# david-cortes/poismf

Hardware: AMD Instinct MI355X
Metric: nonzeros/sec per full A+B sweep (higher is better)
Workload: dtype f32; 1 GPU; uniform 1000000x100000, 99949803 nnz (100000000 triplets, seed 1, duplicates summed), k=50, method=pg, maxupd=10, l2=1000, step=1e-09

## Files before the change

poismf_amd/csrc/poismf_hip.hip:

```cpp
#include <hip/hip_runtime.h>

#include <algorithm>
#include <atomic>
#include <cstdio>
#include <cstdlib>
#include <type_traits>

#include "plan.hpp"
#include "reg_eval.hpp"
#include "quad_eval.hpp"
#include "lane_eval.hpp"
#include "solvers.hpp"

#ifndef PMF_TU
#define PMF_TU -1
#endif
constexpr bool tu_has(int kmethod) { return PMF_TU == -1 || PMF_TU == kmethod; }

template <class EV, class = void> struct cold_constants : std::false_type {};
template <class EV> struct cold_constants<EV, std::void_t<decltype(EV::COLD_CONSTANTS)>> : std::integral_constant<bool, EV::COLD_CONSTANTS> {};

template <class EV, class = void> struct has_idle_tile : std::false_type {};
template <class EV> struct has_idle_tile<EV, std::void_t<decltype(&EV::idle_tile)>> : std::true_type {};

template <class EV, class T, int NC, int METHOD>
__device__ __forceinline__ void solve_row(const HalfArgs<T>& a, EV& ev, const T (&bs)[NC], unsigned lrow, unsigned nnz)
{
    const int k = a.geom.k;
    T* out = a.M + (size_t)(a.row_offset + lrow) * (size_t)k;
    T* out_p = a.Mp != nullptr ? a.Mp + (size_t)(a.row_offset + lrow) * (size_t)a.ldM : nullptr;
    T x[NC];
    if (nnz == 0) {
        T z = (T)0;
        asm volatile("" : "+v"(z));
        PMF_EW x[i] = z;
        ev.store_vec(out, x);
        if (out_p != nullptr) ev.store_vec(out_p, x);
        return;
    }
    ev.start_point(out, x);
    ev.n_eval = 0;

    T shift[NC];
    PMF_EW shift[i] = bs[i];
    const bool weighted = a.P.w != (T)1;
    if (weighted) {
        T cs[NC];
        PMF_EW cs[i] = (T)0;
        ev.tile_colsum(cs);
        T w_here = a.P.w;
        asm volatile("" : "+v"(w_here));
        const T wm1 = w_here - (T)1.;
        PMF_EW {
            shift[i] = cs[i] * wm1;
            shift[i] = shift[i] + bs[i];
        }
        if (METHOD == K_PG) {
            PMF_EW shift[i] = shift[i] * a.P.neg_step;
            if (a.P.neg_step2 != (T)1) { PMF_EW shift[i] = shift[i] * a.P.neg_step2; }
        }
    }

    SolveStats st;
    if constexpr (METHOD == K_EVAL) {
        T g[NC];
        double f;
        if (a.P.maxupd == 0) {
            f = (double)fun_single(ev, a.P, shift, x);
            grad_single(ev, a.P, shift, x, g, weighted);
        } else f = (double)fun_and_grad(ev, a.P, shift, x, g);
        ev.store_vec(out, g);
        if (out_p != nullptr) ev.store_vec(out_p, g);
        if (a.dec_rows != nullptr && ev.lane == 0 && ev.wid == 0 && ev.member == 0) {
            const unsigned long long fb = __builtin_bit_cast(unsigned long long, f);
            a.dec_rows[2 * (size_t)lrow] = (unsigned)fb;
            a.dec_rows[2 * (size_t)lrow + 1] = (unsigned)(fb >> 32);
        }
        return;
    } else if constexpr (METHOD == K_PG) {
        pg_row(ev, a.P, x, shift);
    } else if constexpr (METHOD == K_CG) {
        if constexpr (EV::MAY_CACHE) {
            if (a.P.limit_step && ev.pq_cap > 0 && nnz <= (unsigned)ev.pq_cap) cg_row_cached(ev, a.P, shift, x, weighted, st);
            else cg_row(ev, a.P, shift, x, weighted, st);
        } else cg_row(ev, a.P, shift, x, weighted, st);
    } else {
        T prev[NC];
        PMF_EW prev[i] = x[i];
        if (!a.reuse_prev) { PMF_EW x[i] = (T)1e-3; }
        (void)Tnc<T, NC, EV>::minimize(ev, a.P, shift, x, st);
        if (a.early_stop) {
            PMF_EW prev[i] = prev[i] - x[i];
            const T moved = ev.dot(prev, prev);
            if ((double)moved <= 1e-4 && ev.lane == 0 && ev.wid == 0 && ev.member == 0) atomicAdd(a.n_unchanged, 1u);
        }
    }
    ev.store_vec(out, x);
    if (out_p != nullptr) ev.store_vec(out_p, x);
#ifndef PMF_PROBE
    if (a.eval_rows != nullptr && ev.lane == 0 && ev.wid == 0 && ev.member == 0) a.eval_rows[lrow] += ev.n_eval;
#endif
    if (a.dec_rows != nullptr && ev.lane == 0 && ev.wid == 0 && ev.member == 0) {
        unsigned d0 = (unsigned)st.niter | ((unsigned)st.rc << 24), d1 = (unsigned)st.nfeval;
        if constexpr (cold_constants<EV>::value) asm volatile("" : "+v"(d0), "+v"(d1));
        a.dec_rows[2 * (size_t)lrow] = d0;
        a.dec_rows[2 * (size_t)lrow + 1] = d1;
    }
}

template <int METHOD, class T> __device__ __forceinline__ unsigned take_ticket(const HalfArgs<T>& a)
{
    unsigned st = 0u;
    if constexpr (METHOD != K_PG) {
        if (a.stop != nullptr) st = __hip_atomic_load(a.stop, __ATOMIC_RELAXED, __HIP_MEMORY_SCOPE_SYSTEM);
    }
    const unsigned t = atomicAdd(a.queue, 1u);
    return st != 0u ? 0xffffffffu : t;
}

template <class EV, class T, int NC, int METHOD, int NW>
__device__ __forceinline__ void sweep_rows(const HalfArgs<T>& a, EV& ev, unsigned char* smem)
{
    if (a.gate != nullptr && __hip_atomic_load(a.gate, __ATOMIC_RELAXED, __HIP_MEMORY_SCOPE_AGENT) == 0) return;
    ev.init(a.geom, a.F, smem);
    T bs[NC];
    ev.load_vec(a.bsum, bs);
    const RowDesc* desc = a.desc + a.perm_begin;
    if constexpr (EV::PIPELINED && (EV::PIPE_MW == 1 || (EV::PIPE_MW == 2 && METHOD == K_PG))) {
        unsigned r = blockIdx.x;
        auto ticket = [&]() -> unsigned {
            if (a.queue != nullptr) {
                if constexpr (NW > 1) {
                    unsigned* slot = ev.ticket_slot();
                    if (threadIdx.x == 0) *slot = take_ticket<METHOD>(a);
                    __syncthreads();
                    const unsigned t = uniform(*slot);
                    __syncthreads();
                    return t;
                }
                unsigned t = 0;
                if (ev.lane == 0) t = take_ticket<METHOD>(a);
                return uniform(t);
            }
            unsigned t = r;
            r += gridDim.x;
            if constexpr (METHOD != K_PG) {
                if (a.stop != nullptr && __hip_atomic_load(a.stop, __ATOMIC_RELAXED, __HIP_MEMORY_SCOPE_SYSTEM) != 0u) t = 0xffffffffu;
            }
            return t;
        };
        auto fetch = [&](unsigned t) -> RowDesc { return desc[t < a.nrows ? t : 0u]; };
        unsigned t0 = ticket(), t1 = ticket();
        RowDesc d0 = fetch(t0), d1 = fetch(t1);
        if (t0 < a.nrows) ev.fetch_meta(a.indices + (((unsigned long long)d0.p0_hi << 32) | d0.p0_lo), d0.nnz);
#ifdef PMF_PROBE
        unsigned probe_i = 0;
#endif
        while (t0 < a.nrows) {
            const unsigned long long p0 = ((unsigned long long)d0.p0_hi << 32) | d0.p0_lo;
            if (d0.nnz != 0) ev.gather(a.values + p0, d0.nnz);
            else if constexpr (has_idle_tile<EV>::value) ev.idle_tile();
            const unsigned t2 = ticket();
            const RowDesc d2 = fetch(t2);
            if (t1 < a.nrows) ev.fetch_meta(a.indices + (((unsigned long long)d1.p0_hi << 32) | d1.p0_lo), d1.nnz);
#ifdef PMF_PROBE
            ev.probe = (a.eval_rows != nullptr && blockIdx.x == 5 && threadIdx.x < WAVE && probe_i < 60) ? a.eval_rows + 16 * probe_i : nullptr;
            if (ev.probe != nullptr && ev.lane == 0) { ev.probe[10] = (unsigned)__builtin_amdgcn_s_memtime(); ev.probe[11] = d0.nnz; }
            probe_i++;
#endif
            solve_row<EV, T, NC, METHOD>(a, ev, bs, d0.lrow, d0.nnz);
            t0 = t1; d0 = d1;
            t1 = t2; d1 = d2;
        }
        return;
    } else {
        unsigned r = blockIdx.x;
        for (;;) {
            if (a.queue != nullptr) {
                if constexpr (NW > 1) {
                    unsigned* next_row = ev.ticket_slot();
                    if (threadIdx.x == 0) *next_row = take_ticket<METHOD>(a);
                    __syncthreads();
                    r = uniform(*next_row);
                    __syncthreads();
                } else {
                    unsigned t = 0;
                    if (ev.lane == 0) t = take_ticket<METHOD>(a);
                    r = uniform(t);
                }
            }
            if (r >= a.nrows) break;
            if constexpr (METHOD != K_PG) {
                if (a.queue == nullptr && a.stop != nullptr && uniform(__hip_atomic_load(a.stop, __ATOMIC_RELAXED, __HIP_MEMORY_SCOPE_SYSTEM)) != 0u) break;
            }
            const RowDesc d = desc[r];
            r += gridDim.x;
            const unsigned nnz = uniform(d.nnz);
            const unsigned long long p0 = ((unsigned long long)uniform(d.p0_hi) << 32) | uniform(d.p0_lo);
            if (nnz != 0) ev.begin_row(a.indices + p0, a.values + p0, nnz);
            solve_row<EV, T, NC, METHOD>(a, ev, bs, uniform(d.lrow), nnz);
        }
    }
}

template <class T, int NC, int METHOD, int SL, int NW>
__global__ __launch_bounds__(WAVE* NW) void half_sweep_kernel(const HalfArgs<T> a)
{
    extern __shared__ __attribute__((aligned(16))) unsigned char smem[];
    constexpr bool PF = SL > 0 && METHOD != K_TNCG;
    RowEval<T, NC, SL, NW, PF> ev;
    if constexpr (NW > 1) {
        if (a.arrive != nullptr && threadIdx.x == 0) atomicAdd(a.arrive, 1u);
    }
#ifdef PMF_TIMING
    const unsigned long long t_kernel = __builtin_amdgcn_s_memtime();
#endif
    sweep_rows<RowEval<T, NC, SL, NW, PF>, T, NC, METHOD, NW>(a, ev, smem);
#ifdef PMF_TIMING
    ev.tacc[5] = __builtin_amdgcn_s_memtime() - t_kernel;
    if (ev.lane == 0 && ev.wid == 0)
        for (int q = 0; q < 6; q++) atomicAdd(&g_pmf_timing[q], ev.tacc[q]);
#endif
}

template <class EV, class T, int NC, int METHOD>
__device__ __forceinline__ void team_rows(const HalfArgs<T>& a, EV& ev, unsigned char* smem)
{
    if (a.arrive != nullptr && threadIdx.x == 0) atomicAdd(a.arrive, 1u);
    ev.init(a.geom, a.F, smem);
    T bs[NC];
    ev.load_vec(a.bsum, bs);
    const RowDesc* desc = a.desc + a.perm_begin;
    const unsigned M = a.team_members;
    unsigned* box = ev.ticket_slot();
    if (threadIdx.x == 0) {
        const unsigned n = atomicAdd((unsigned*)a.team_buf, 1u);
        box[0] = n / M;
        box[1] = n % M;
    }
    __syncthreads();
    const unsigned team = uniform(box[0]);
    ev.member = (int)uniform(box[1]);
    __syncthreads();
    if ((size_t)(team + 1) * gt_team_words(M) + GT_HEAD_WORDS > GT_BUF_BYTES / 8) return;
    ev.tm_M = (int)M;
    ev.tm_seq = 0;
    ev.tm_words = a.team_buf + GT_HEAD_WORDS + (size_t)team * gt_team_words(M);
    ev.tm_err = a.team_err;
    ev.tm_spin = a.team_spin;
    unsigned long long* mail = ev.tm_words;
    constexpr unsigned END = 0xffffffffu;
    if (threadIdx.x == 0) atomicAdd((unsigned*)(mail + 2), 1u);
    if (a.team_spin <= 1u && threadIdx.x == 0) __hip_atomic_store(a.team_err, 1u, __ATOMIC_RELAXED, __HIP_MEMORY_SCOPE_AGENT);
    if (ev.wid == 0) {
        for (unsigned spins = 0;; spins++) {
            if (a.team_spin <= 1u) break;
            if (uniform((unsigned)gt_load(mail + 2)) >= M) break;
            if ((spins & 255u) == 255u) {
                if (uniform(__hip_atomic_load(a.team_err, __ATOMIC_RELAXED, __HIP_MEMORY_SCOPE_AGENT)) != 0) break;
                if (uniform(__hip_atomic_load(a.queue, __ATOMIC_RELAXED, __HIP_MEMORY_SCOPE_AGENT)) >= a.nrows) break;
            }
            if ((spins >> 6) > a.team_spin) { __hip_atomic_store(a.team_err, 1u, __ATOMIC_RELAXED, __HIP_MEMORY_SCOPE_AGENT); break; }
            __builtin_amdgcn_s_sleep(8);
        }
    }
    __syncthreads();
    for (unsigned rowno = 1;; rowno++) {
        if (ev.wid == 0) {
            unsigned tk = END;
            if (ev.member == 0) {
                unsigned t0 = 0;
                if (ev.lane == 0) t0 = take_ticket<METHOD>(a);
                tk = uniform(t0);
                if (tk >= a.nrows || uniform(__hip_atomic_load(a.team_err, __ATOMIC_RELAXED, __HIP_MEMORY_SCOPE_AGENT)) != 0) tk = END;
                gt_store(mail + (rowno & 1u), ((unsigned long long)rowno << 32) | tk);
            } else {
                unsigned seen = uniform(__hip_atomic_load(a.queue, __ATOMIC_RELAXED, __HIP_MEMORY_SCOPE_AGENT));
                for (unsigned spins = 0;; spins++) {
                    const unsigned long long v = gt_load(mail + (rowno & 1u));
                    const unsigned hi = uniform((unsigned)(v >> 32)), lo = uniform((unsigned)v);
                    if (hi == rowno) { tk = lo; break; }
                    if ((spins & 255u) == 255u) {
                        if (uniform(__hip_atomic_load(a.team_err, __ATOMIC_RELAXED, __HIP_MEMORY_SCOPE_AGENT)) != 0) break;
                        const unsigned q = uniform(__hip_atomic_load(a.queue, __ATOMIC_RELAXED, __HIP_MEMORY_SCOPE_AGENT));
                        if (q != seen) { seen = q; spins = 0; }
                        else if (rowno == 1u && q >= a.nrows) break;
                    }
                    if (spins > a.team_spin) { __hip_atomic_store(a.team_err, 1u, __ATOMIC_RELAXED, __HIP_MEMORY_SCOPE_AGENT); break; }
                    __builtin_amdgcn_s_sleep(4);
                }
            }
            box[0] = tk;
        }
        __syncthreads();
        const unsigned t = uniform(box[0]);
        __syncthreads();
        if (t >= a.nrows) break;
        const RowDesc d = desc[t];
        const unsigned nnz = uniform(d.nnz);
        const unsigned long long p0 = ((unsigned long long)uniform(d.p0_hi) << 32) | uniform(d.p0_lo);
        const unsigned S = ((nnz + M - 1u) / M + (EV::TEAM_ROUND - 1u)) / EV::TEAM_ROUND * EV::TEAM_ROUND;
        const unsigned off = (unsigned)ev.member * S;
        const unsigned mine = off < nnz ? (nnz - off < S ? nnz - off : S) : 0u;
        ev.begin_row(a.indices + p0 + (mine ? off : 0u), a.values + p0 + (mine ? off : 0u), mine);
        solve_row<EV, T, NC, METHOD>(a, ev, bs, uniform(d.lrow), nnz);
    }
}
template <class T, int NC, int METHOD, int SL, int NW>
__global__ __launch_bounds__(WAVE* NW) void half_sweep_giant_kernel(const HalfArgs<T> a)
{
    extern __shared__ __attribute__((aligned(16))) unsigned char smem[];
    constexpr bool PF = SL > 0 && METHOD != K_TNCG;
    using EV = RowEval<T, NC, SL, NW, PF, true>;
    EV ev;
    team_rows<EV, T, NC, METHOD>(a, ev, smem);
}
template <class T, int METHOD, int KS, int LV, int LA, int LL, int NW, int LP>
__global__ __launch_bounds__(WAVE* NW) __attribute__((amdgpu_waves_per_eu(1, 1))) void half_sweep_lane_team_kernel(const HalfArgs<T> a)
{
    using EV = LaneEval<T, KS, LV, LA, LL, NW, false, LP, 0, true>;
    __shared__ __attribute__((aligned(16))) unsigned char smem[EV::SMEM_BYTES];
    EV ev;
    team_rows<EV, T, EV::NC, METHOD>(a, ev, smem);
}

#ifndef PMF_PG_EXTRA
#define PMF_PG_EXTRA 56
#endif
#ifndef PMF_CG_EXTRA
#define PMF_CG_EXTRA 120
#endif
#ifndef PMF_TNC_EXTRA
#define PMF_TNC_EXTRA 100
#endif
constexpr int reg_waves(int tile_regs, int method)
{
    const int need = tile_regs + (method == K_PG ? PMF_PG_EXTRA : method == K_CG ? PMF_CG_EXTRA : PMF_TNC_EXTRA);
    for (int w : { 8, 6, 5, 4, 3, 2 })
        if ((512 / w) / 8 * 8 >= need) return w;
    return 1;
}
template <class T, int METHOD, int G, int NS> constexpr bool reg_pairs() { return METHOD == K_PG && sizeof(T) == 4 && G == 16 && NS == 1; }
template <class T, int METHOD, int S, int G, int NS>
__global__ __launch_bounds__(WAVE) __attribute__((amdgpu_waves_per_eu(reg_waves(4 * S * NS, METHOD)))) void half_sweep_reg_kernel(const HalfArgs<T> a)
{
    using EV = RegEval<T, S, G, NS, 1, 1, reg_pairs<T, METHOD, G, NS>()>;
    EV ev;
    constexpr int SMEM = EV::SMEM_BYTES;
    __shared__ __attribute__((aligned(16))) unsigned char smem[SMEM > 0 && METHOD == K_CG ? SMEM : 16];
#ifdef PMF_TIMING
    const unsigned long long t_kernel = __builtin_amdgcn_s_memtime();
#endif
    sweep_rows<EV, T, EV::NC, METHOD, 1>(a, ev, smem);
#ifdef PMF_TIMING
    if (ev.lane == 0) atomicAdd(&g_pmf_timing[5], __builtin_amdgcn_s_memtime() - t_kernel);
#endif
}

template <int Q>
__global__ __launch_bounds__(WAVE) __attribute__((amdgpu_waves_per_eu(reg_waves(QuadEval<Q>::TILE_REGS, K_PG)))) void half_sweep_quad_kernel(const HalfArgs<float> a)
{
    using EV = QuadEval<Q>;
    EV ev;
    sweep_rows<EV, float, EV::NC, K_PG, 1>(a, ev, nullptr);
}

constexpr int regw_waves(int tile_regs, int method, int nw)
{
    const int w = reg_waves(tile_regs + (method == K_PG ? 8 : 0), method);
    return nw >= 16 && w < 4 ? 4 : (nw >= 8 && w < 2 ? 2 : w);
}
template <class T, int METHOD, int S, int G, int NS, int NW>
__global__ __launch_bounds__(WAVE* NW) __attribute__((amdgpu_waves_per_eu(regw_waves(4 * S * NS, METHOD, NW)))) void half_sweep_regw_kernel(const HalfArgs<T> a)
{
    using EV = RegEval<T, S, G, NS, NW>;
    __shared__ __attribute__((aligned(16))) unsigned char smem[EV::SMEM_BYTES];
    EV ev;
    sweep_rows<EV, T, EV::NC, METHOD, NW>(a, ev, smem);
}

template <class T, int METHOD, int S, int G, int NS, int NW, int M>
__global__ __launch_bounds__(WAVE* NW) __attribute__((amdgpu_waves_per_eu(1))) void half_sweep_team_kernel(const HalfArgs<T> a)
{
    using EV = RegEval<T, S, G, NS, NW, M>;
    constexpr int NC = EV::NC;
    __shared__ __attribute__((aligned(16))) unsigned char smem[EV::SMEM_BYTES];
    EV ev;
    ev.init(a.geom, a.F, smem);
    T bs[NC];
    ev.load_vec(a.bsum, bs);
    const RowDesc* desc = a.desc + a.perm_begin;
    unsigned* arrive = (unsigned*)a.team_buf;
    unsigned* err = a.team_err;
    unsigned* box = ev.ticket_slot();
    if (threadIdx.x == 0) {
        unsigned xcc = 0;
        if (gridDim.x >= 8u * 4u * (unsigned)M) {
            asm volatile("s_getreg_b32 %0, hwreg(HW_REG_XCC_ID)" : "=s"(xcc));
            xcc &= 7u;
        }
        const unsigned n = atomicAdd(arrive + xcc, 1u);
        box[0] = xcc * TEAM_SLOTS_PER_XCD + n / (unsigned)M;
        box[1] = n % (unsigned)M;
        if (n / (unsigned)M >= TEAM_SLOTS_PER_XCD) __hip_atomic_store(err, 2u, __ATOMIC_RELAXED, __HIP_MEMORY_SCOPE_AGENT);
    }
    __syncthreads();
    const unsigned team = uniform(box[0]) % TEAM_SLOTS;
    ev.member = (int)uniform(box[1]);
    __syncthreads();
    ev.team_words = a.team_buf + TEAM_HEAD_WORDS + (size_t)team * TEAM_WORDS;
    ev.team_err = err;
    ev.team_spin = a.team_spin;
    unsigned long long* mail = ev.team_words;
    unsigned long long* here = ev.team_words + 2;
    constexpr unsigned END = 0xffffffffu;
    if (ev.member != 0 && threadIdx.x == 0) gran_store(here + ev.member, 1ull);

    if (ev.member == 0) {
        if (threadIdx.x == 0) {
            unsigned full = 0;
            unsigned seen = __hip_atomic_load(a.queue, __ATOMIC_RELAXED, __HIP_MEMORY_SCOPE_AGENT);
            for (unsigned spins = 0; !full; spins++) {
                full = 1;
                for (int m = 1; m < M; m++) full &= gran_load(here + m) != 0ull;
                if (full) break;
                const unsigned q = __hip_atomic_load(a.queue, __ATOMIC_RELAXED, __HIP_MEMORY_SCOPE_AGENT);
                if (q >= a.nrows || __hip_atomic_load(err, __ATOMIC_RELAXED, __HIP_MEMORY_SCOPE_AGENT) != 0) break;
                if (q != seen) { seen = q; spins = 0; }
                if (spins > a.team_spin) { __hip_atomic_store(err, 3u, __ATOMIC_RELAXED, __HIP_MEMORY_SCOPE_AGENT); break; }
                __builtin_amdgcn_s_sleep(8);
            }
            box[0] = full;
        }
        __syncthreads();
        const bool full = uniform(box[0]) != 0;
        __syncthreads();
        if (!full) {
            if (threadIdx.x == 0) gran_store(mail + 1, ((unsigned long long)1u << 32) | END);
            return;
        }
    }

    auto next_ticket = [&](unsigned rowno_next) -> unsigned {
        if (ev.member == 0) {
            if (threadIdx.x == 0) {
                box[0] = take_ticket<METHOD>(a);
                gran_store(mail + (rowno_next & 1u), ((unsigned long long)rowno_next << 32) | (box[0] < a.nrows ? box[0] : END));
            }
        } else if (threadIdx.x == 0) {
            unsigned long long v = 0;
            unsigned seen = __hip_atomic_load(a.queue, __ATOMIC_RELAXED, __HIP_MEMORY_SCOPE_AGENT);
            for (unsigned spins = 0;; spins++) {
                v = gran_load(mail + (rowno_next & 1u));
                if ((unsigned)(v >> 32) == rowno_next) break;
                if ((spins & 255u) == 255u) {
                    if (__hip_atomic_load(err, __ATOMIC_RELAXED, __HIP_MEMORY_SCOPE_AGENT) != 0) { v = END; break; }
                    const unsigned q = __hip_atomic_load(a.queue, __ATOMIC_RELAXED, __HIP_MEMORY_SCOPE_AGENT);
                    if (rowno_next == 1u && q != seen) { seen = q; spins = 0; }
                }
                if (spins > a.team_spin) {
                    __hip_atomic_store(err, 1u, __ATOMIC_RELAXED, __HIP_MEMORY_SCOPE_AGENT);
                    v = END;
                    break;
                }
                __builtin_amdgcn_s_sleep(2);
            }
            box[0] = (unsigned)v;
        }
        __syncthreads();
        const unsigned tk = uniform(box[0]);
        __syncthreads();
        return tk;
    };
    auto row_of = [&](unsigned tk, unsigned& nnz, unsigned long long& p0, unsigned& lrow) {
        const RowDesc d = desc[tk < a.nrows ? tk : 0u];
        nnz = uniform(d.nnz);
        p0 = ((unsigned long long)uniform(d.p0_hi) << 32) | uniform(d.p0_lo);
        lrow = uniform(d.lrow);
    };
    unsigned rowno = 1;
    unsigned t = next_ticket(1);
    unsigned nnz = 0, lrow = 0;
    unsigned long long p0 = 0;
    row_of(t, nnz, p0, lrow);
    if (t < a.nrows) ev.fetch_meta(a.indices + p0, nnz);
    while (t < a.nrows) {
        if (__hip_atomic_load(err, __ATOMIC_RELAXED, __HIP_MEMORY_SCOPE_AGENT) != 0) break;
#ifdef PMF_PROBE
        const unsigned long long t_row0 = __builtin_amdgcn_s_memtime();
        ev.probe_wait = 0;
#endif
        ev.gather(a.values + p0, nnz);
        const unsigned t_next = next_ticket(rowno + 1);
        unsigned nnz_next = 0, lrow_next = 0;
        unsigned long long p0_next = 0;
        row_of(t_next, nnz_next, p0_next, lrow_next);
        if (t_next < a.nrows) ev.fetch_meta(a.indices + p0_next, nnz_next);
#ifdef PMF_PROBE
        {
            T probe_sum[NC];
            PMF_EW probe_sum[i] = (T)0;
            ev.tile_touch(probe_sum);
            ev.probe_acc[4] += __builtin_amdgcn_s_memtime() - t_row0;
            if (probe_sum[0] == (T)123.456) ev.probe_acc[6]++;
        }
#endif
        solve_row<EV, T, NC, METHOD>(a, ev, bs, lrow, nnz);
#ifdef PMF_PROBE
        if (a.eval_rows != nullptr && threadIdx.x == 0 && ev.member == 0)
            a.eval_rows[lrow] = (unsigned)std::min<unsigned long long>(0xffffu, ev.probe_wait >> 8) |
                                ((unsigned)std::min<unsigned long long>(0xffffu, (__builtin_amdgcn_s_memtime() - t_row0) >> 8) << 16);
        ev.probe_acc[5] += __builtin_amdgcn_s_memtime() - t_row0;
        ev.probe_acc[6] += ev.probe_wait;
#endif
        rowno++;
        t = t_next; nnz = nnz_next; p0 = p0_next; lrow = lrow_next;
    }
#ifdef PMF_PROBE
    if (threadIdx.x == 0 && ev.member == 0)
        for (int q = 0; q < 8; q++) atomicAdd(a.team_buf + 8 + q, ev.probe_acc[q]);
#endif
}

template <bool SMALL> constexpr bool lane_two() { return SMALL; }
template <class T, int METHOD, int KS, int LV, int LA, int LL, int NW, bool SMALL, int LP = 0, int TX = 0, int KU = 0>
__global__ __launch_bounds__(WAVE* NW) __attribute__((amdgpu_waves_per_eu(lane_two<SMALL>() ? 2 : 1, lane_two<SMALL>() ? 2 : 1))) void half_sweep_lane_kernel(const HalfArgs<T> a)
{
    using EV = LaneEval<T, KS, LV, LA, LL, NW, SMALL, LP, TX, false, KU>;
    __shared__ __attribute__((aligned(16))) unsigned char smem[EV::SMEM_BYTES];
    EV ev;
    sweep_rows<EV, T, EV::NC, METHOD, NW>(a, ev, smem);
}

namespace {

using std::integral_constant;
constexpr int MAX_DEVICES = 64;

template <auto Kern, int THREADS> int launch_grid(const OneLaunch& o, const HalfArgs<real_t>& a, unsigned grid, size_t lds = 0)
{
    if (o.dry) return 0;
    hipLaunchKernelGGL(Kern, dim3(grid), dim3(THREADS), lds, o.stream, a);
    HIP_TRY(hipGetLastError());
    return 0;
}
template <auto Kern, int THREADS> int launch_occ(const OneLaunch& o, const HalfArgs<real_t>& a)
{
    if (o.dry) return 0;
    static std::atomic<int> occ_cache{0};
    int occ = occ_cache.load(std::memory_order_relaxed);
    if (occ == 0) {
        int n = 0;
        HIP_TRY(hipOccupancyMaxActiveBlocksPerMultiprocessor(&n, reinterpret_cast<const void*>(Kern), THREADS, 0));
        occ = std::max(1, n);
        occ_cache.store(occ, std::memory_order_relaxed);
    }
    return launch_grid<Kern, THREADS>(o, a, (unsigned)std::min<size_t>(a.nrows, (size_t)o.num_cu * (size_t)occ * o.grid_mult));
}
template <auto Kern, int THREADS> int launch_lds(const OneLaunch& o, const HalfArgs<real_t>& a)
{
    if (o.dry) return 0;
    static std::atomic<bool> attr_set[MAX_DEVICES];
    const int dev = o.device >= 0 && o.device < MAX_DEVICES ? o.device : 0;
    if (!attr_set[dev].load(std::memory_order_acquire) || dev != o.device) {
        HIP_TRY(hipFuncSetAttribute(reinterpret_cast<const void*>(Kern), hipFuncAttributeMaxDynamicSharedMemorySize, (int)LDS_PER_CU));
        attr_set[dev].store(true, std::memory_order_release);
    }
    return launch_grid<Kern, THREADS>(o, a, o.grid, o.lds);
}

template <class F> int with_method(int method, F f)
{
    switch (method) {
        case POISMF_PG:
            if constexpr (tu_has(K_PG)) return f(integral_constant<int, K_PG>{});
            else return 1;
        case POISMF_CG:
            if constexpr (tu_has(K_CG)) return f(integral_constant<int, K_CG>{});
            else return 1;
        case POISMF_EVAL:
            if constexpr (tu_has(K_EVAL)) return f(integral_constant<int, K_EVAL>{});
            else return 1;
        default:
            if constexpr (tu_has(K_TNCG)) return f(integral_constant<int, K_TNCG>{});
            else return 1;
    }
}
template <class F> int with_steps(int S, F f)
{
    switch (S) {
#define X(NZ) case (NZ) / REG_JG: return f(integral_constant<int, (NZ) / REG_JG>{});
        PMF_REG_SIZES(X)
#undef X
    }
    return 1;
}
template <class F> int with_slots(const OneLaunch& o, F f)
{
    if (o.s_load == SPECIAL_SL_A) return f(integral_constant<int, SLOT_ELEMS>{}, integral_constant<int, SPECIAL_SL_A>{});
    if (o.s_load == SPECIAL_SL_B) return f(integral_constant<int, SLOT_ELEMS>{}, integral_constant<int, SPECIAL_SL_B>{});
    switch (o.spl) {
        case 1: return f(integral_constant<int, 1 * SLOT_ELEMS>{}, integral_constant<int, 0>{});
        case 2: return f(integral_constant<int, 2 * SLOT_ELEMS>{}, integral_constant<int, 0>{});
    }
    return 1;
}

template <int NW> int launch_bin(int method, const OneLaunch& o, const HalfArgs<real_t>& a)
{
    return with_slots(o, [&](auto nc, auto sl) {
        return with_method(method, [&](auto m) {
            return launch_lds<half_sweep_kernel<real_t, decltype(nc)::value, decltype(m)::value, decltype(sl)::value, NW>, WAVE * NW>(o, a);
        });
    });
}
int launch_giant(int method, const OneLaunch& o, const HalfArgs<real_t>& a)
{
    return with_slots(o, [&](auto nc, auto sl) {
        if constexpr (tu_has(K_TNCG)) {
            if (method == POISMF_TNCG)
                return launch_lds<half_sweep_giant_kernel<real_t, decltype(nc)::value, K_TNCG, decltype(sl)::value, LONG_NW>, WAVE * LONG_NW>(o, a);
        }
        return 1;
    });
}

int launch_reg(int method, const OneLaunch& o, const HalfArgs<real_t>& a)
{
    return with_method(method, [&](auto m) {
        return with_steps(o.reg_S, [&](auto s) {
            constexpr int M = decltype(m)::value, S = decltype(s)::value;
            const int ns = REG_NS_MAX == 1 || o.s_load <= REG_G ? 1 : 2;
            if constexpr (reg_instance(M, S, 1)) {
                if (ns == 1) return launch_occ<half_sweep_reg_kernel<real_t, M, S, REG_G, 1>, WAVE>(o, a);
            }
            if constexpr (reg_instance(M, S, 2)) {
                if (ns == 2) return launch_occ<half_sweep_reg_kernel<real_t, M, S, REG_G, 2>, WAVE>(o, a);
            }
            return 1;
        });
    });
}
int launch_quad(int method, const OneLaunch& o, const HalfArgs<real_t>& a)
{
    if (method != POISMF_PG || a.geom.k != QUAD_K || a.geom.ldF != QUAD_LD) return 1;
    return with_steps(o.reg_S, [&](auto s) {
        if constexpr (tu_has(K_PG) && sizeof(real_t) == 4 && PMF_REG_QUAD != 0 && REG_G == 16)
            return launch_occ<half_sweep_quad_kernel<decltype(s)::value * REG_JG / 16>, WAVE>(o, a);
        else return 1;
    });
}
template <int NW> int launch_regw(int method, const OneLaunch& o, const HalfArgs<real_t>& a)
{
    return with_method(method, [&](auto m) {
        return with_steps(o.reg_S, [&](auto s) {
            constexpr int M = decltype(m)::value, S = decltype(s)::value;
            if constexpr (regw_instance(M, S, NW)) {
                if (REG_G == 16 || o.s_load <= REG_G) return launch_occ<half_sweep_regw_kernel<real_t, M, S, REG_G, 1, NW>, WAVE * NW>(o, a);
                if constexpr (REG_G != 16) return launch_occ<half_sweep_regw_kernel<real_t, M, S, REG_G, 2, NW>, WAVE * NW>(o, a);
            }
            return 1;
        });
    });
}
template <int M, int S> int launch_team(int method, const OneLaunch& o, const HalfArgs<real_t>& a)
{
    if constexpr ((tu_has(K_CG) || tu_has(K_EVAL)) && sizeof(real_t) == 8 && REG_G == 16) {
        constexpr int KM = tu_has(K_CG) ? K_CG : K_EVAL;
        if (method != (KM == K_CG ? POISMF_CG : POISMF_EVAL)) return 1;
        const unsigned grid = (unsigned)std::min<size_t>((size_t)a.nrows * M, (size_t)o.num_cu / M * M);
        return launch_grid<half_sweep_team_kernel<real_t, KM, S, REG_G, 2, TEAM_NW, M>, WAVE * TEAM_NW>(o, a, grid);
    } else return 1;
}

template <int METHOD, int KS, int LV, int LA, int LL, int NW, bool SMALL, int LP, int TX, int KU> int launch_lane(const OneLaunch& o, const HalfArgs<real_t>& a)
{
    using EV = LaneEval<real_t, KS, LV, LA, LL, NW, SMALL, LP, TX, false, KU>;
    const int occ = std::max(1, std::min((lane_two<SMALL>() ? 8 : 4) / NW, (int)(LDS_PER_CU / (size_t)EV::SMEM_BYTES)));
    const unsigned grid = (unsigned)std::min<size_t>(a.nrows, (size_t)o.num_cu * (size_t)occ * o.grid_mult);
    return launch_grid<half_sweep_lane_kernel<real_t, METHOD, KS, LV, LA, LL, NW, SMALL, LP, TX, KU>, WAVE * NW>(o, a, grid);
}
int launch_lane_shape(int method, const OneLaunch& o, const HalfArgs<real_t>& a)
{
    return with_method(method, [&](auto m) {
        constexpr int M = decltype(m)::value;
#define X(FOR, KS, LV, LA, LL, NW, SMALL, LP, TX, KU)                                                  \
        if constexpr ((((FOR) >> M) & 1u) != 0 && ((KU) == 0 || PMF_LANE_KU50 != 0)) {                 \
            if (o.s_load == (KS) && o.lane == LaneShape{ LV, LA, LL, NW, SMALL, LP, TX, KU })          \
                return launch_lane<M, KS, LV, LA, LL, NW, (SMALL) != 0, LP, TX, KU>(o, a);             \
        }
        PMF_LANE_INSTANCES(X)
#undef X
        return 1;
    });
}
int launch_lane_team(int method, const OneLaunch& o, const HalfArgs<real_t>& a)
{
    return with_method(method, [&](auto m) {
        if constexpr (decltype(m)::value == K_TNCG && sizeof(real_t) == 8) {
            if (o.s_load == LANE_TEAM_KS && o.lane == LANE_TEAM_SHAPE)
                return launch_grid<half_sweep_lane_team_kernel<real_t, K_TNCG, LANE_TEAM_KS, LANE_TEAM_SHAPE.lv, LANE_TEAM_SHAPE.la, LANE_TEAM_SHAPE.ll, LANE_TEAM_SHAPE.waves,
                                                               LANE_TEAM_SHAPE.lp>, WAVE * LANE_TEAM_SHAPE.waves>(o, a, o.grid);
        }
        return 1;
    });
}

int launch_one_here(int method, const OneLaunch& o, const HalfArgs<real_t>& a)
{
    switch (o.engine) {
        case Engine::LaneTeam: return launch_lane_team(method, o, a);
        case Engine::Lane: return launch_lane_shape(method, o, a);
#ifndef PMF_LANE_ONLY
        case Engine::RegTeam:
#define X(M, S) if (o.team == (M) && o.reg_S == (S)) return launch_team<M, S>(method, o, a);
            PMF_TEAM_SHAPES(X)
#undef X
            return 1;
        case Engine::Reg: return o.quad != 0 ? launch_quad(method, o, a) : launch_reg(method, o, a);
        case Engine::RegW:
            switch (o.nw) {
                case 2: return launch_regw<2>(method, o, a);
                case 4: return launch_regw<4>(method, o, a);
                case 8: return launch_regw<8>(method, o, a);
            }
            return 1;
        case Engine::Giant: return launch_giant(method, o, a);
        case Engine::LdsLong: return launch_bin<LONG_NW>(method, o, a);
        case Engine::Lds: return launch_bin<1>(method, o, a);
#else
        default: return 1;
#endif
    }
    return 1;
}
}

#if PMF_TU == 1 || PMF_TU == -1
int pmf_launch_one_tu1(int method, const OneLaunch& o, const HalfArgs<real_t>& a) { return launch_one_here(method, o, a); }
#endif
#if PMF_TU == 2 || PMF_TU == -1
int pmf_launch_one_tu2(int method, const OneLaunch& o, const HalfArgs<real_t>& a) { return launch_one_here(method, o, a); }
#endif
#if PMF_TU == 3 || PMF_TU == -1
int pmf_launch_one_tu3(int method, const OneLaunch& o, const HalfArgs<real_t>& a) { return launch_one_here(method, o, a); }
#endif
#if PMF_TU == 4 || PMF_TU == -1
int pmf_launch_one_tu4(int method, const OneLaunch& o, const HalfArgs<real_t>& a) { return launch_one_here(method, o, a); }
#endif

#ifdef PMF_TIMING
int pmf_read_timing(unsigned long long* out)
{
    (void)hipDeviceSynchronize();
    if (hipMemcpyFromSymbol(out, HIP_SYMBOL(g_pmf_timing), sizeof(unsigned long long) * 8) != hipSuccess) return 1;
    unsigned long long z[8] = {0, 0, 0, 0, 0, 0, 0, 0};
    return hipMemcpyToSymbol(HIP_SYMBOL(g_pmf_timing), z, sizeof(z)) != hipSuccess;
}
#endif
```

poismf_amd/csrc/quad_eval.hpp:

```cpp
#pragma once
#include "reg_eval.hpp"

namespace pmf {

#define PMF_QFOLD4(Q, A, B) \
    "v_add_f32_dpp " Q ", " A ", " A " row_shl:4 row_mask:0xf bank_mask:0x5\n\t" \
    "v_add_f32_dpp " Q ", " B ", " B " row_shr:4 row_mask:0xf bank_mask:0xa\n\t"
__device__ __forceinline__ void quad_fold14(const float (&p)[14], float (&q)[7])
{
    asm("s_nop 1\n\t"
        PMF_QFOLD4("%0", "%7", "%14")
        PMF_QFOLD4("%1", "%8", "%15")
        PMF_QFOLD4("%2", "%9", "%16")
        PMF_QFOLD4("%3", "%10", "%17")
        PMF_QFOLD4("%4", "%11", "%18")
        PMF_QFOLD4("%5", "%12", "%19")
        PMF_QFOLD4("%6", "%13", "%20")
        : "=&v"(q[0]), "=&v"(q[1]), "=&v"(q[2]), "=&v"(q[3]), "=&v"(q[4]), "=&v"(q[5]), "=&v"(q[6])
        : "v"(p[0]), "v"(p[1]), "v"(p[2]), "v"(p[3]), "v"(p[4]), "v"(p[5]), "v"(p[6]),
          "v"(p[7]), "v"(p[8]), "v"(p[9]), "v"(p[10]), "v"(p[11]), "v"(p[12]), "v"(p[13]));
}
__device__ __forceinline__ void quad_fold7(const float (&q)[7], float (&r)[4])
{
    asm("s_nop 1\n\t"
        PMF_FOLD2("row_ror:8", "0x3", "0xc", "%0", "%4", "%8")
        PMF_FOLD2("row_ror:8", "0x3", "0xc", "%1", "%5", "%9")
        PMF_FOLD2("row_ror:8", "0x3", "0xc", "%2", "%6", "%10")
        PMF_FOLD1("row_ror:8", "%3", "%7")
        : "=&v"(r[0]), "=&v"(r[1]), "=&v"(r[2]), "=&v"(r[3])
        : "v"(q[0]), "v"(q[1]), "v"(q[2]), "v"(q[3]), "v"(q[4]), "v"(q[5]), "v"(q[6]));
}
__device__ __forceinline__ float quad_tail_sum(float g)
{
    asm("s_nop 1\n\t"
        "v_add_f32_dpp %0, %0, %0 quad_perm:[1,0,3,2] row_mask:0x6 bank_mask:0x8\n\t"
        "s_nop 1\n\t"
        "v_add_f32_dpp %0, %0, %0 quad_perm:[2,3,0,1] row_mask:0x6 bank_mask:0x8"
        : "+v"(g));
    return g;
}

template <int Q> struct QuadEval {
    using T = float;
    static_assert(Q >= 1 && Q <= 10, "one to ten steps of sixteen nonzeros");
    typedef float V2 __attribute__((ext_vector_type(2)));
    struct __attribute__((packed, aligned(4))) U4 { float v[4]; };
    struct __attribute__((packed, aligned(4))) U2 { float v[2]; };
    static constexpr int K = 50;
    static constexpr int NP = 6;
    static constexpr int NA = NP + 1;
    static constexpr int NE = 2 * NA;
    static constexpr int NC = 1;
    static constexpr int NB = (Q + 3) / 4;
    static constexpr int TILE_REGS = 2 * NP * Q + 2 * NB;
    static constexpr int NW = 1, M = 1;
    static constexpr bool PIPELINED = true;
    static constexpr int PIPE_MW = 1;
    static constexpr bool FUSED_SUMS = false, PREFETCH = false, MAY_CACHE = false, CACHED_GRAD = false;
    static constexpr bool PG_LEAN = true;
    static constexpr int SMEM_BYTES = 0;
    static_assert(K == 4 * 2 * NP + 2, "four lanes of twelve elements and a tail of two");

    V2 t[Q][NP];
    V2 tt[NB];
    V2 a[NA];
    T xr[NB];
    unsigned idx_n[NB];
    const T* F;
    unsigned zero_row;
    int k, ldF;
    int lane, q, wid, member;
    int jlane;
    int dim;
    bool primary;
    bool cls1, cls2, cls16, cls32;
    int xor32_addr;
    int quad_addr;
    unsigned nnz;
    unsigned n_eval;
#ifdef PMF_PROBE
    unsigned* probe = nullptr;
#endif

    static __host__ __device__ constexpr int acc_of(int quad)
    {
        const int n = ((quad >> 3) & 1) + 2 * ((quad >> 2) & 1) + 4 * ((quad >> 1) & 1);
        return (n == 7 ? 3 : n) + 7 * (quad & 1);
    }
    static __host__ __device__ constexpr int quad_of(int e)
    {
        const int n = e % 7;
        return (e / 7) + 2 * ((n >> 2) & 1) + 4 * ((n >> 1) & 1) + 8 * (n & 1);
    }
    static __host__ __device__ constexpr int dim_of(int q_, int e) { return e < 2 * NP ? 2 * NP * q_ + e : 8 * NP + (e - 2 * NP); }

    __device__ __forceinline__ void init(const TileGeom& geo, const T* F_, unsigned char*)
    {
        lane = lane_id();
        F = F_;
        k = geo.k; ldF = geo.ldF; zero_row = geo.zero_row;
        q = lane & 3; wid = 0; member = 0;
        jlane = 16 * q + (lane >> 2);
        cls1 = (lane & 1) != 0; cls2 = (lane & 2) != 0; cls16 = (lane & 16) != 0; cls32 = (lane & 32) != 0;
        const int quad = lane >> 2;
        const int e = acc_of(quad);
        dim = dim_of(q, e);
        primary = (quad >> 1) != 7 && (e < 2 * NP || q == 0);
        xor32_addr = (lane ^ 32) << 2;
        quad_addr = q << 2;
        asm volatile("" : "+v"(xor32_addr), "+v"(quad_addr));
    }

    __device__ __forceinline__ void load_vec(const T* p, T (&x)[NC]) const { x[0] = p[dim]; }
    __device__ __forceinline__ void start_point(const T* mrow, T (&x)[NC]) const { load_vec(mrow, x); }
    __device__ __forceinline__ void store_vec(T* p, const T (&x)[NC]) const
    {
        if (primary) p[dim] = x[0];
    }

    __device__ __forceinline__ void fetch_meta(const unsigned* ind, unsigned nnz_row)
    {
#pragma unroll
        for (int b = 0; b < NB; b++) {
            const unsigned j = (unsigned)(64 * b + jlane);
            idx_n[b] = j < nnz_row ? ind[j] : zero_row;
        }
    }
    __device__ __forceinline__ void begin_row(const unsigned* ind, const T* val, unsigned nnz_row)
    {
        fetch_meta(ind, nnz_row);
        gather(val, nnz_row);
    }
    __device__ __forceinline__ unsigned* ticket_slot() const { return nullptr; }
    __device__ __forceinline__ void gather(const T* val, unsigned nnz_row)
    {
        nnz = nnz_row;
        unsigned idx[NB];
#pragma unroll
        for (int b = 0; b < NB; b++) {
            const unsigned j = (unsigned)(64 * b + jlane);
            idx[b] = idx_n[b];
            xr[b] = j < nnz ? val[j] : (T)0;
        }
        const unsigned rowbytes = (unsigned)ldF * (unsigned)sizeof(T);
        const unsigned main_off = (unsigned)q * 48u;
#pragma unroll
        for (int b = 0; b < NB; b++) tt[b] = (V2){ (T)0, (T)0 };
        static_for<0, Q>([&](auto sc) {
            constexpr int s = decltype(sc)::value;
            const unsigned c = group_bcast<4, s % 4>(idx[s / 4]);
            const char* base = (const char*)F + (size_t)(__umul24(c, rowbytes) + main_off);
            const U4 v0 = *(const U4*)base;
            const U4 v1 = *(const U4*)(base + 16);
            const U4 v2 = *(const U4*)(base + 32);
            t[s][0] = (V2){ v0.v[0], v0.v[1] }; t[s][1] = (V2){ v0.v[2], v0.v[3] };
            t[s][2] = (V2){ v1.v[0], v1.v[1] }; t[s][3] = (V2){ v1.v[2], v1.v[3] };
            t[s][4] = (V2){ v2.v[0], v2.v[1] }; t[s][5] = (V2){ v2.v[2], v2.v[3] };
            if (q == s % 4) {
                const U2 w = *(const U2*)((const char*)F + (size_t)(__umul24(idx[s / 4], rowbytes) + 192u));
                tt[s / 4] = (V2){ w.v[0], w.v[1] };
            }
        });
    }
    __device__ __forceinline__ void idle_tile()
    {
        asm volatile("" ::: "memory");
#pragma unroll
        for (int s = 0; s < Q; s++) {
#pragma unroll
            for (int e = 0; e < NP; e++) t[s][e] = (V2){ (T)0, (T)0 };
        }
#pragma unroll
        for (int b = 0; b < NB; b++) tt[b] = (V2){ (T)0, (T)0 };
    }

    __device__ __forceinline__ void set_point_as_is(const T (&x)[NC])
    {
#define PMF_QPERM(D, E) "ds_bpermute_b32 " D ", %14, %15 offset:%" E "\n\t"
        float r[NE];
        asm volatile(PMF_QPERM("%0", "16") PMF_QPERM("%1", "17") PMF_QPERM("%2", "18") PMF_QPERM("%3", "19") PMF_QPERM("%4", "20")
                     PMF_QPERM("%5", "21") PMF_QPERM("%6", "22") PMF_QPERM("%7", "23") PMF_QPERM("%8", "24") PMF_QPERM("%9", "25")
                     PMF_QPERM("%10", "26") PMF_QPERM("%11", "27") PMF_QPERM("%12", "28") PMF_QPERM("%13", "29")
                     "s_waitcnt lgkmcnt(0)"
                     : "=&v"(r[0]), "=&v"(r[1]), "=&v"(r[2]), "=&v"(r[3]), "=&v"(r[4]), "=&v"(r[5]), "=&v"(r[6]), "=&v"(r[7]), "=&v"(r[8]), "=&v"(r[9]),
                       "=&v"(r[10]), "=&v"(r[11]), "=&v"(r[12]), "=&v"(r[13])
                     : "v"(quad_addr), "v"(x[0]), "n"(16 * quad_of(0)), "n"(16 * quad_of(1)), "n"(16 * quad_of(2)), "n"(16 * quad_of(3)),
                       "n"(16 * quad_of(4)), "n"(16 * quad_of(5)), "n"(16 * quad_of(6)), "n"(16 * quad_of(7)), "n"(16 * quad_of(8)), "n"(16 * quad_of(9)),
                       "n"(16 * quad_of(10)), "n"(16 * quad_of(11)), "n"(16 * quad_of(12)), "n"(16 * quad_of(13)));
#undef PMF_QPERM
#pragma unroll
        for (int e = 0; e < NA; e++) a[e] = (V2){ r[2 * e], r[2 * e + 1] };
    }
    __device__ __forceinline__ void set_point(const T (&x)[NC]) { set_point_as_is(x); }

    template <int N> __device__ __forceinline__ T quad_transpose_sum(const T (&p)[4]) const
    {
        T r0, r1;
        if constexpr (N >= 2) r0 = fold_pair<0xB1>(cls1, p[0], p[1]);
        else r0 = fold_one<0xB1>(p[0]);
        if constexpr (N == 4) r1 = fold_pair<0xB1>(cls1, p[2], p[3]);
        else if constexpr (N == 3) r1 = fold_one<0xB1>(p[2]);
        if constexpr (N >= 3) return fold_pair<0x4E>(cls2, r0, r1);
        else return fold_one<0x4E>(r0);
    }

    __device__ __forceinline__ T cross_quads(const T (&part)[NE]) const
    {
        T l4[7], l8[4];
        quad_fold14(part, l4);
        quad_fold7(l4, l8);
        T l16[2];
#pragma unroll
        for (int i = 0; i < 2; i++) {
            const T own = cls16 ? l8[i + 2] : l8[i];
            const T send = cls16 ? l8[i] : l8[i + 2];
            l16[i] = own + __builtin_bit_cast(T, __builtin_amdgcn_ds_swizzle(__builtin_bit_cast(int, send), 0x401f));
        }
        const T own = cls32 ? l16[1] : l16[0];
        const T send = cls32 ? l16[0] : l16[1];
        static_assert(quad_of(2 * NP) == 11 && quad_of(2 * NP + 1) == 7, "quad_tail_sum's masks: DPP rows 2 and 1, bank 3");
        return quad_tail_sum(own + __builtin_bit_cast(T, __builtin_amdgcn_ds_bpermute(xor32_addr, __builtin_bit_cast(int, send))));
    }

    template <bool WANT_F, bool WANT_G, bool FROM_CACHE = false, bool FRESH = false> __device__ __forceinline__ double eval(T sgn, T (&acc)[NC], T* = nullptr)
    {
        static_assert(!WANT_F && WANT_G && !FROM_CACHE, "the quad engine evaluates PG's gradient only");
        n_eval++;
        PMF_STAMP(*this, 0);
        V2 part2[NA];
        static_for<0, NB>([&](auto bc) {
            constexpr int b = decltype(bc)::value;
            constexpr int n = (Q - 4 * b) < 4 ? (Q - 4 * b) : 4;
            T p[4];
            V2 s2[n];
#pragma unroll
            for (int u = 0; u < n; u++) s2[u] = t[4 * b + u][0] * a[0];
#pragma unroll
            for (int e = 1; e < NP; e++) {
#pragma unroll
                for (int u = 0; u < n; u++) s2[u] = __builtin_elementwise_fma(t[4 * b + u][e], a[e], s2[u]);
            }
#pragma unroll
            for (int u = 0; u < 4; u++) p[u] = u < n ? s2[u < n ? u : 0].x + s2[u < n ? u : 0].y : (T)0;
            T pred = quad_transpose_sum<n>(p);
            pred = __builtin_fmaf(tt[b].x, a[NP].x, __builtin_fmaf(tt[b].y, a[NP].y, pred));
            const bool on = (unsigned)(64 * b + jlane) < nnz;
            const T coef = on ? coef_div(sgn * xr[b], pred) : (T)0;
            {
                const V2 c2 = { coef, coef };
                if constexpr (b == 0) part2[NP] = c2 * tt[0];
                else part2[NP] = __builtin_elementwise_fma(c2, tt[b], part2[NP]);
            }
            static_for<0, n>([&](auto uc) {
                constexpr int u = decltype(uc)::value;
                const T c = group_bcast<4, u>(coef);
                const V2 c2 = { c, c };
#pragma unroll
                for (int e = 0; e < NP; e++) {
                    if constexpr (b == 0 && u == 0) part2[e] = c2 * t[0][e];
                    else part2[e] = __builtin_elementwise_fma(c2, t[4 * b + u][e], part2[e]);
                }
            });
        });
        PMF_STAMP(*this, 5);
        T part[NE];
#pragma unroll
        for (int e = 0; e < NA; e++) { part[2 * e] = part2[e].x; part[2 * e + 1] = part2[e].y; }
        const T g = cross_quads(part);
        acc[0] = FRESH ? g : acc[0] + g;
        PMF_STAMP(*this, 6);
        return 0.0;
    }

    __device__ __forceinline__ void tile_colsum(T (&acc)[NC])
    {
        T part[NE];
#pragma unroll
        for (int i = 0; i < NE; i++) part[i] = (T)0;
#pragma unroll
        for (int s = 0; s < Q; s++) {
#pragma unroll
            for (int e = 0; e < NP; e++) { part[2 * e] += t[s][e].x; part[2 * e + 1] += t[s][e].y; }
        }
#pragma unroll
        for (int b = 0; b < NB; b++) { part[2 * NP] += tt[b].x; part[2 * NP + 1] += tt[b].y; }
        acc[0] += cross_quads(part);
    }
};

}
```

Measured before the change: 12.60 billion nnz/s.

## Park per-lane bsum and output offset in LDS to cut quad kernel VGPRs

Measured after the change: 12.31 billion nnz/s. 2.3% lower.

```diff
diff --git a/poismf_amd/csrc/poismf_hip.hip b/poismf_amd/csrc/poismf_hip.hip
--- a/poismf_amd/csrc/poismf_hip.hip
+++ b/poismf_amd/csrc/poismf_hip.hip
@@ -19,6 +19,9 @@
 
 template <class EV, class = void> struct cold_constants : std::false_type {};
 template <class EV> struct cold_constants<EV, std::void_t<decltype(EV::COLD_CONSTANTS)>> : std::integral_constant<bool, EV::COLD_CONSTANTS> {};
+
+template <class EV, class = void> struct parks_bsum : std::false_type {};
+template <class EV> struct parks_bsum<EV, std::void_t<decltype(EV::PARKED)>> : std::integral_constant<bool, EV::PARKED> {};
 
 template <class EV, class = void> struct has_idle_tile : std::false_type {};
 template <class EV> struct has_idle_tile<EV, std::void_t<decltype(&EV::idle_tile)>> : std::true_type {};
@@ -38,11 +41,16 @@
         if (out_p != nullptr) ev.store_vec(out_p, x);
         return;
     }
-    ev.start_point(out, x);
+    T bsr[NC];
+    if constexpr (parks_bsum<EV>::value) ev.start_point(out, x, bsr);
+    else {
+        ev.start_point(out, x);
+        PMF_EW bsr[i] = bs[i];
+    }
     ev.n_eval = 0;
 
     T shift[NC];
-    PMF_EW shift[i] = bs[i];
+    PMF_EW shift[i] = bsr[i];
     const bool weighted = a.P.w != (T)1;
     if (weighted) {
         T cs[NC];
@@ -53,7 +61,7 @@
         const T wm1 = w_here - (T)1.;
         PMF_EW {
             shift[i] = cs[i] * wm1;
-            shift[i] = shift[i] + bs[i];
+            shift[i] = shift[i] + bsr[i];
         }
         if (METHOD == K_PG) {
             PMF_EW shift[i] = shift[i] * a.P.neg_step;
@@ -125,6 +133,7 @@
     ev.init(a.geom, a.F, smem);
     T bs[NC];
     ev.load_vec(a.bsum, bs);
+    if constexpr (parks_bsum<EV>::value) ev.park(bs);
     const RowDesc* desc = a.desc + a.perm_begin;
     if constexpr (EV::PIPELINED && (EV::PIPE_MW == 1 || (EV::PIPE_MW == 2 && METHOD == K_PG))) {
         unsigned r = blockIdx.x;
@@ -333,12 +342,15 @@
 #ifndef PMF_TNC_EXTRA
 #define PMF_TNC_EXTRA 100
 #endif
-constexpr int reg_waves(int tile_regs, int method)
-{
-    const int need = tile_regs + (method == K_PG ? PMF_PG_EXTRA : method == K_CG ? PMF_CG_EXTRA : PMF_TNC_EXTRA);
+constexpr int waves_for(int need)
+{
     for (int w : { 8, 6, 5, 4, 3, 2 })
         if ((512 / w) / 8 * 8 >= need) return w;
     return 1;
+}
+constexpr int reg_waves(int tile_regs, int method)
+{
+    return waves_for(tile_regs + (method == K_PG ? PMF_PG_EXTRA : method == K_CG ? PMF_CG_EXTRA : PMF_TNC_EXTRA));
 }
 template <class T, int METHOD, int G, int NS> constexpr bool reg_pairs() { return METHOD == K_PG && sizeof(T) == 4 && G == 16 && NS == 1; }
 template <class T, int METHOD, int S, int G, int NS>
@@ -358,11 +370,14 @@
 }
 
 template <int Q>
-__global__ __launch_bounds__(WAVE) __attribute__((amdgpu_waves_per_eu(reg_waves(QuadEval<Q>::TILE_REGS, K_PG)))) void half_sweep_quad_kernel(const HalfArgs<float> a)
+__global__ __launch_bounds__(WAVE) __attribute__((amdgpu_waves_per_eu(waves_for(QuadEval<Q>::TILE_REGS + QuadEval<Q>::WORK_REGS)))) void half_sweep_quad_kernel(const HalfArgs<float> a)
 {
     using EV = QuadEval<Q>;
     EV ev;
-    sweep_rows<EV, float, EV::NC, K_PG, 1>(a, ev, nullptr);
+    if constexpr (EV::SMEM_BYTES > 0) {
+        __shared__ __attribute__((aligned(16))) unsigned char smem[EV::SMEM_BYTES];
+        sweep_rows<EV, float, EV::NC, K_PG, 1>(a, ev, smem);
+    } else sweep_rows<EV, float, EV::NC, K_PG, 1>(a, ev, nullptr);
 }
 
 constexpr int regw_waves(int tile_regs, int method, int nw)
diff --git a/poismf_amd/csrc/quad_eval.hpp b/poismf_amd/csrc/quad_eval.hpp
--- a/poismf_amd/csrc/quad_eval.hpp
+++ b/poismf_amd/csrc/quad_eval.hpp
@@ -58,7 +58,10 @@
     static constexpr int PIPE_MW = 1;
     static constexpr bool FUSED_SUMS = false, PREFETCH = false, MAY_CACHE = false, CACHED_GRAD = false;
     static constexpr bool PG_LEAN = true;
-    static constexpr int SMEM_BYTES = 0;
+    static constexpr bool PARKED = Q == 7 || Q == 9;
+    static constexpr bool COLD_CONSTANTS = PARKED;
+    static constexpr int WORK_REGS = PARKED ? 40 : 56;
+    static constexpr int SMEM_BYTES = PARKED ? 2 * 4 * WAVE : 0;
     static_assert(K == 4 * 2 * NP + 2, "four lanes of twelve elements and a tail of two");
 
     V2 t[Q][NP];
@@ -67,6 +70,7 @@
     T xr[NB];
     unsigned idx_n[NB];
     const T* F;
+    unsigned char* smem;
     unsigned zero_row;
     int k, ldF;
     int lane, q, wid, member;
@@ -94,8 +98,9 @@
     }
     static __host__ __device__ constexpr int dim_of(int q_, int e) { return e < 2 * NP ? 2 * NP * q_ + e : 8 * NP + (e - 2 * NP); }
 
-    __device__ __forceinline__ void init(const TileGeom& geo, const T* F_, unsigned char*)
-    {
+    __device__ __forceinline__ void init(const TileGeom& geo, const T* F_, unsigned char* smem_)
+    {
+        smem = smem_;
         lane = lane_id();
         F = F_;
         k = geo.k; ldF = geo.ldF; zero_row = geo.zero_row;
@@ -111,18 +116,46 @@
         asm volatile("" : "+v"(xor32_addr), "+v"(quad_addr));
     }
 
+    __device__ __forceinline__ int jl() const
+    {
+        if constexpr (PARKED) return (int)(((unsigned)quad_addr << 2) | (((unsigned)xor32_addr >> 4) ^ 8u));
+        else return jlane;
+    }
+    __device__ __forceinline__ unsigned main_offset() const
+    {
+        if constexpr (PARKED) return (unsigned)quad_addr * 12u;
+        else return (unsigned)q * 48u;
+    }
+    __device__ __forceinline__ unsigned* slot() const { return (unsigned*)(smem + xor32_addr); }
+    __device__ __forceinline__ void park(const T (&bs)[NC]) const
+    {
+        slot()[0] = (unsigned)dim * (unsigned)sizeof(T);
+        slot()[WAVE] = __builtin_bit_cast(unsigned, bs[0]);
+    }
+
     __device__ __forceinline__ void load_vec(const T* p, T (&x)[NC]) const { x[0] = p[dim]; }
     __device__ __forceinline__ void start_point(const T* mrow, T (&x)[NC]) const { load_vec(mrow, x); }
+    __device__ __forceinline__ void start_point(const T* mrow, T (&x)[NC], T (&bs)[NC]) const
+    {
+        const unsigned off = slot()[0];
+        bs[0] = __builtin_bit_cast(T, slot()[WAVE]);
+        x[0] = *(const T*)((const char*)mrow + off);
+    }
     __device__ __forceinline__ void store_vec(T* p, const T (&x)[NC]) const
     {
-        if (primary) p[dim] = x[0];
+        if constexpr (PARKED) {
+            const unsigned off = slot()[0];
+            if (primary) *(T*)((char*)p + off) = x[0];
+        } else {
+            if (primary) p[dim] = x[0];
+        }
     }
 
     __device__ __forceinline__ void fetch_meta(const unsigned* ind, unsigned nnz_row)
     {
 #pragma unroll
         for (int b = 0; b < NB; b++) {
-            const unsigned j = (unsigned)(64 * b + jlane);
+            const unsigned j = (unsigned)(64 * b + jl());
             idx_n[b] = j < nnz_row ? ind[j] : zero_row;
         }
     }
@@ -135,15 +168,16 @@
     __device__ __forceinline__ void gather(const T* val, unsigned nnz_row)
     {
         nnz = nnz_row;
+        if constexpr (PARKED) asm volatile("" : "+v"(xor32_addr), "+v"(quad_addr));
         unsigned idx[NB];
 #pragma unroll
         for (int b = 0; b < NB; b++) {
-            const unsigned j = (unsigned)(64 * b + jlane);
+            const unsigned j = (unsigned)(64 * b + jl());
             idx[b] = idx_n[b];
             xr[b] = j < nnz ? val[j] : (T)0;
         }
         const unsigned rowbytes = (unsigned)ldF * (unsigned)sizeof(T);
-        const unsigned main_off = (unsigned)q * 48u;
+        const unsigned main_off = main_offset();
 #pragma unroll
         for (int b = 0; b < NB; b++) tt[b] = (V2){ (T)0, (T)0 };
         static_for<0, Q>([&](auto sc) {
@@ -244,7 +278,7 @@
             for (int u = 0; u < 4; u++) p[u] = u < n ? s2[u < n ? u : 0].x + s2[u < n ? u : 0].y : (T)0;
             T pred = quad_transpose_sum<n>(p);
             pred = __builtin_fmaf(tt[b].x, a[NP].x, __builtin_fmaf(tt[b].y, a[NP].y, pred));
-            const bool on = (unsigned)(64 * b + jlane) < nnz;
+            const bool on = (unsigned)(64 * b + jl()) < nnz;
             const T coef = on ? coef_div(sgn * xr[b], pred) : (T)0;
             {
                 const V2 c2 = { coef, coef };
```
